# cohensbw/ElPhDynamics

Measured on AMD Instinct MI355X. Metric: cg_matvecs_per_sec, higher is better.
Workload: dtype f64; 1 GPU; BASELINE config C: Holstein square L=16 Ntau=160 (N=256, Ltau=160, Ndim=40960), un-preconditioned CG iteration, 288 right-hand sides per step on each GPU = 144 independent Markov chain(s) x 2 solve(s) each (2 = the two pseudofermion solves of one HMC force evaluation), 1 GPU(s) with their own chains; nrhs=288, chains_per_gpu=144, ndim=40960, preconditioned=False, form=workgroup-resident: K iterations of the whole batch in one launch (k_cg_wg), parallelism=gpus1xchains144

## Files before the change

elphdynamics_amd/csrc/cg_wg.hip:

```cpp

#include <algorithm>
#include <atomic>
#include <type_traits>

#include "cg_fast_common.h"

#include "cg_wg_dev.h"
#include "pgrid_dev.h"

namespace wg {

#ifdef ELPH_WG_ARRIVE
__device__ unsigned long long g_wg_arrive[4096 * 4];
__device__ unsigned long long g_wg_timeline[4096 * 4];
#define TL(k) do { if (threadIdx.x == 0 && blockIdx.x < 4096) g_wg_timeline[blockIdx.x * 4 + (k)] = (unsigned long long)wall_clock64(); } while (0)
#else
#define TL(k) do { } while (0)
#endif

struct WgRankArgs { CgBufs B; ModelDev m; WgCtl R; ShardCtl Sh; };
template <int NPL, int T, bool SSH, bool UNI, int FORM, bool SHARD, bool X0Z = false, bool RANKS = false>
__global__ void __launch_bounds__(512) k_cg_wg(CgBufs B, ModelDev m, WgCtl R, ShardCtl Sh) {
    static_assert(!RANKS || SHARD, "several ranks per launch: sharded solves only");
    unsigned bid = 0;
// ... 55 lines not shown
    double *eall = rall + (size_t)(X_REG ? 1 : 2) * W * T * HSL;
    double *el = eall + (size_t)wv * (E_SHARED ? T : T + 1) * HSL;
    double *partA = eall + (E_LDS ? (E_SHARED ? ((size_t)W * T + 1) * HSL : (size_t)W * (T + 1) * HSL) : (S_LDS ? (size_t)W * SQ_TABS * WAVE : 0)), *partB = partA + 8, *bc = partA + 16;
    double *part = partA, *tot = partA + 32, *partF = partA + 40, *rhalo = partA + 48, *zhalo = rhalo + 2 * HSL;
    double *phl = zhalo + 2 * HSL + (size_t)wv * 2 * HSL;
#define PHALO(k, q) phl[((k) ? 1 : 0) * HSL + lr + (q) * LSL]
    auto wrap = [L](int t) { return (t < 0) ? t + L : ((t >= L) ? t - L : t); };
    auto sgn = [](int t) { return (t == 0) ? -1.0 : 1.0; };
    const CgParams P = B.params;
    CgState *st2 = B.state + 2 * rhs;
    const CgState S = ld_state(st2);
    if (!SHARD && (S.done || S.seq != 0)) return;

    int sc[NPL], ss[NPL];
    bool live[NPL], own[NPL];
#pragma unroll
    for (int q = 0; q < NPL; ++q) {
        const int s = SQ ? sq_patch_site(lane, q) : (HC ? hc_site(lane, q) : (S8 ? s8_site(lane) : (GR ? grid_site(lane, q, GGX, GGY) : (HG ? hgrid_site<NPL>(lane, q, HLX, HLY) : lane + q * WAVE))));
        live[q] = (GR || HG) ? lwok : (REGX || s < N);
        own[q] = SHARD ? (live[q] && s >= Sh.own_lo && s < Sh.own_hi) : (HC ? hc_real(lane) : live[q]);
        sc[q] = live[q] ? s : N - 1;
        ss[q] = live[q] ? s : N;
    }
    double *xg = B.x + (size_t)rhs * ndim, *rg = B.r + (size_t)rhs * ndim;
    const double *Ech = m.E + (size_t)(rhs % m.nchains) * m.E_chain_stride;

    double zw[T + 1][NPL], p[T + 2][NPL], E[E_LDS ? 1 : NEJ][NPL], xr[X_REG ? T : 1][NPL];
#pragma unroll
    for (int j = 0; j < T; ++j)
#pragma unroll
        for (int q = 0; q < NPL; ++q) {
            if (lwok) rl[j * HSL + lr + q * LSL] = rg[(size_t)(t0 + j) * N + sc[q]];
            if (X_GLB) {}
            else if (X_REG) xr[X_REG ? j : 0][q] = X0Z ? 0.0 : xg[(size_t)(t0 + j) * N + sc[q]];
            else if (lwok) xl[j * HSL + lr + q * LSL] = X0Z ? 0.0 : xg[(size_t)(t0 + j) * N + sc[q]];
        }
#pragma unroll
    for (int j = 0; j < T + 2; ++j)
#pragma unroll
        for (int q = 0; q < NPL; ++q) {
            p[j][q] = rg[(size_t)wrap(t0 + j - 1) * N + sc[q]];
            if (PH_LDS && (j == 0 || j == T + 1) && lwok) PHALO(j, q) = p[j][q];
        }
#pragma unroll
    for (int j = 0; j < NEJ; ++j)
#pragma unroll
        for (int q = 0; q < NPL; ++q) {
            const double ev = Ech[(size_t)wrap(t0 + j) * m.E_tau_stride + sc[q]];
            if (E_LDS) { if (lwok) el[j * HSL + lr + q * LSL] = ev; }
            else E[E_LDS ? 0 : j][q] = ev;
        }
    unsigned ij[NE];
    Tab<NE, UNI> tab[NT];
    SqCtx<UNI> X;
    SqSsh<NSREG, S_LDS> XS;
    HcCtx XH;
    S8Ctx X8;
    GridCtx XG;
    HgCtx XHG;
    pgrid::Ctx XT;
    if constexpr (GR) {
        XG = grid_ctx(lane, GGX, GGY, m.c_uni, m.s_uni);
        if constexpr (TG) { XT = pgrid::Tri<2, 2>::make_ctx(lane, 2 * GGX, m.c_uni, m.s_uni); XG.k4 = XT.ks; }
    } else if constexpr (HG) {
        XHG = hgrid_ctx<NPL>(lane, HLX, HLY, m.c_uni, m.s_uni);
    } else if constexpr (S8) {
        X8.th = m.s_uni / m.c_uni; X8.k4 = (m.c_uni * m.c_uni) * (m.c_uni * m.c_uni);
        X8.yx = sq_patch_ycross(lane); X8.xodd = (lane >> 1) & 1;
    } else if constexpr (HC) {
        XH.th = m.s_uni / m.c_uni; XH.k3 = m.c_uni * m.c_uni * m.c_uni;
        XH.up = (lane + 16) & (WAVE - 1); XH.dn = (lane + 48) & (WAVE - 1);
    } else if constexpr (SQ && SSH) {
        ssh_chain_select(m, rhs);
        XS.yx = sq_patch_ycross(lane);
        XS.l0 = eall + (size_t)wv * SQ_TABS * WAVE + lane;
#pragma unroll
        for (int j = 0; j <= T; ++j) {
            const double *cj = m.c + (size_t)wrap(t0 + j) * m.cs_tau_stride, *sj = m.s + (size_t)wrap(t0 + j) * m.cs_tau_stride;
            SqTabS tb;
#pragma unroll
            for (int pr = 0; pr < 2; ++pr) {
                const int b0 = m.sq_bond[0 * N + sc[2 * pr]], b2 = m.sq_bond[2 * N + sc[pr]];
                tb.ci[0][pr] = cj[b0]; tb.si[0][pr] = sj[b0];
                tb.ci[1][pr] = cj[b2]; tb.si[1][pr] = sj[b2];
            }
#pragma unroll
            for (int k = 0; k < 4; ++k) {
                const int b1 = m.sq_bond[1 * N + sc[k]], b3 = m.sq_bond[3 * N + sc[k]];
                tb.cx[0][k] = cj[b1]; tb.sx[0][k] = sj[b1];
                tb.cx[1][k] = cj[b3]; tb.sx[1][k] = sj[b3];
            }
            if (S_LDS && j == 0) {
                double *d = eall + (size_t)wv * SQ_TABS * WAVE + lane;
#pragma unroll
                for (int pr = 0; pr < 2; ++pr) {
                    d[(0 + pr) * WAVE] = tb.ci[0][pr]; d[(2 + pr) * WAVE] = tb.si[0][pr];
                    d[(4 + pr) * WAVE] = tb.ci[1][pr]; d[(6 + pr) * WAVE] = tb.si[1][pr];
                }
#pragma unroll
                for (int k = 0; k < 4; ++k) {
                    d[(8 + k) * WAVE] = tb.cx[0][k]; d[(12 + k) * WAVE] = tb.sx[0][k];
                    d[(16 + k) * WAVE] = tb.cx[1][k]; d[(20 + k) * WAVE] = tb.sx[1][k];
                }
            } else {
                XS.t[S_LDS ? (j > 0 ? j - 1 : 0) : (j < NSREG ? j : 0)] = tb;
            }
        }
    } else if constexpr (SQ) {
        X.yx = sq_patch_ycross(lane);
        if constexpr (UNI) {
            X.c[0][0] = m.c_uni; X.s[0][0] = m.s_uni / m.c_uni; X.k4 = (m.c_uni * m.c_uni) * (m.c_uni * m.c_uni);
        } else {
            X.k4 = 1.0;
#pragma unroll
            for (int col = 0; col < 4; ++col)
#pragma unroll
                for (int k = 0; k < 4; ++k) {
                    const int bd = m.sq_bond[col * N + sc[k]];
                    X.c[UNI ? 0 : col][UNI ? 0 : k] = m.c[bd];
                    X.s[UNI ? 0 : col][UNI ? 0 : k] = m.s[bd];
                }
        }
    } else {
#pragma unroll
        for (int e = 0; e < NE; ++e) ij[e] = m.lp_ij[e * WAVE + lane];
        if (SSH) {
            ssh_chain_select(m, rhs);
#pragma unroll
            for (int j = 0; j < NT; ++j)
                load_tab<NE, UNI>(tab[j], m.lp_c + (size_t)wrap(t0 + j) * m.lp_tau_stride, m.lp_s + (size_t)wrap(t0 + j) * m.lp_tau_stride, lane, m);
        } else {
            load_tab<NE, UNI>(tab[0], m.lp_c, m.lp_s, lane, m);
        }
    }
#define EXPV(j, q) (E_LDS ? el[(j) * HSL + lr + (q) * LSL] : E[(SSH || E_LDS) ? 0 : (j)][q])

    constexpr size_t SLOTS_RHS = SLOTS_PER_RHS;
    u64 *const slots0 = R.slots + (size_t)rhs * 2 * SLOTS_RHS;
    u64 *const bnd0 = R.bnd + (size_t)rhs * 2 * G * 2 * HS * 2;
    const int gm = (g == 0) ? G - 1 : g - 1, gp = (g == G - 1) ? 0 : g + 1;
    double rho = S.rho, kmin = S.kmin, eps = S.eps;
    double eps0 = S.eps0, normb = S.normb;

    if (threadIdx.x == 0) { tot[5] = 1.0; if (SHARD) bc[2] = 1.0; }
    if (G > 1) {
        if (wv == 0) {
#pragma unroll
            for (int q = 0; q < NPL; ++q) if (lwok) rhalo[lr + q * LSL] = p[0][q];
        }
        if (wv == W - 1) {
#pragma unroll
            for (int q = 0; q < NPL; ++q) if (lwok) rhalo[HSL + lr + q * LSL] = p[T + 1][q];
        }
    }
    const u64 *gaddr[NPL];
    if constexpr (SHARD) {
#pragma unroll
        for (int q = 0; q < NPL; ++q) {
            const int s = ss[q];
            gaddr[q] = (s < Sh.own_lo) ? sh_ghost(Sh.mail[Sh.rank], 0, L, Sh.cap_ghost, t0, s)
                     : (s >= Sh.own_hi && s < N) ? sh_ghost(Sh.mail[Sh.rank], 1, L, Sh.cap_ghost, t0, s - Sh.own_hi) : nullptr;
        }
        double a0 = 0.0;
#pragma unroll
        for (int q = 0; q < NPL; ++q) if (own[q]) a0 += p[1][q] * p[1][q];
        a0 = wave_sum_dpp(a0);
        if (lane == 0) partA[wv] = a0;
        wg_barrier();
        if (wv == 0) {
            const double mine = wg_sum(partA, W, lane);
            sh_publish<RANKS>(Sh, 0, g, G, mine, 1u, lane);
            const u64 *none[NPL];
#pragma unroll
            for (int q = 0; q < NPL; ++q) none[q] = nullptr;
            double tot = 0.0, dummy[NPL];
            const bool ok = sh_poll<NPL, RANKS>(Sh, true, 0, G, none, 1u, lane, R, tot, dummy);
            if (lane == 0) { bc[0] = tot; if (!ok) bc[2] = 0.0; }
        }
        wg_barrier();
        if (bc[2] == 0.0) return;
        const double bb = bc[0];
        normb = sqrt(bb); eps0 = 1.0; eps = 1.0; rho = bb; kmin = 0.0;
        wg_barrier();
    }
    double rr_far = (P.tol * normb) * (P.tol * normb) * 1.000001, y_num = 4.0 * (eps0 * normb) * (eps0 * normb);
    double it_kappa = 0.17 * sqrt(P.kmax);
    constexpr bool FUSED = !SHARD && T >= 2, BSUM = SQ;
    auto uni = [](double v) __attribute__((always_inline)) {
        return __hiloint2double(__builtin_amdgcn_readfirstlane(__double2hiint(v)), __builtin_amdgcn_readfirstlane(__double2loint(v)));
    };
    if constexpr (FUSED) { rr_far = uni(rr_far); y_num = uni(y_num); it_kappa = uni(it_kappa); normb = uni(normb); eps0 = uni(eps0); }
    STAMP_DECL;
    for (long long seq = 0;; ++seq) {
        const unsigned epoch = R.epoch0 + (unsigned)seq + (SHARD ? 2u : 1u);
        const unsigned par = epoch & 1u;
        u64 *const slotsA = slots0 + (size_t)par * SLOTS_RHS, *const slotsB = slotsA + SLOTS_A;
        u64 *const bnd = bnd0 + (size_t)par * G * 2 * HS * 2;
        const size_t ghp = SHARD ? (size_t)par * 2 * L * Sh.cap_ghost * 2 : 0;
        STAMP(9);
        if (seq == 0) TL(0);
        if (seq == 1) TL(1);
        double (&w)[T + 1][NPL] = zw;
        double b_pz = 0.0, b_rz = 0.0, b_zz = 0.0, b_rr = 0.0;
        if constexpr (S8) {
#pragma unroll
            for (int k = 0; k <= T; ++k) w[k][0] = EXPV(k, 0) * p[k][0];
            s8_sweepN<T + 1, false>(w, X8);
#pragma unroll
            for (int k = 0; k <= T; ++k) w[k][0] = p[k + 1][0] - sgn(wrap(t0 + k)) * X8.k4 * w[k][0];
            double gq[T][1];
#pragma unroll
            for (int i = 0; i < T; ++i) gq[i][0] = w[i + 1][0];
            s8_sweepN<T, true>(gq, X8);
#pragma unroll
            for (int i = 0; i < T; ++i) w[i][0] = w[i][0] - sgn(wrap(t0 + i + 1)) * X8.k4 * (EXPV(i + 1, 0) * gq[i][0]);
        } else if constexpr (HC) {
#pragma unroll
            for (int k = 0; k <= T; ++k)
#pragma unroll
                for (int q = 0; q < NPL; ++q) w[k][q] = EXPV(k, q) * ((PH_LDS && k == 0) ? PHALO(0, q) : p[k][q]);
            hc_sweepN<T + 1, false>(w, XH);
#pragma unroll
            for (int k = 0; k <= T; ++k) {
                const double sg = sgn(wrap(t0 + k)) * XH.k3;
#pragma unroll
                for (int q = 0; q < NPL; ++q) w[k][q] = ((PH_LDS && k == T) ? PHALO(1, q) : p[k + 1][q]) - sg * w[k][q];
            }
            auto rev = [&](auto nb, auto j0c) __attribute__((always_inline)) {
                constexpr int NB = decltype(nb)::value, j0 = decltype(j0c)::value;
                double gq[NB][NPL];
#pragma unroll
                for (int i = 0; i < NB; ++i)
#pragma unroll
                    for (int q = 0; q < NPL; ++q) gq[i][q] = w[j0 + i + 1][q];
                hc_sweepN<NB, true>(gq, XH);
#pragma unroll
                for (int i = 0; i < NB; ++i) {
                    const double sg = sgn(wrap(t0 + j0 + i + 1)) * XH.k3;
#pragma unroll
                    for (int q = 0; q < NPL; ++q) w[j0 + i][q] = w[j0 + i][q] - sg * (EXPV(j0 + i + 1, q) * gq[i][q]);
                }
            };
            using std::integral_constant;
            if constexpr (T == 3) { rev(integral_constant<int, 2>(), integral_constant<int, 0>()); rev(integral_constant<int, 1>(), integral_constant<int, 2>()); }
            else rev(integral_constant<int, T>(), integral_constant<int, 0>());
        } else if constexpr (HG) {
#pragma unroll
            for (int k = 0; k <= T; ++k)
#pragma unroll
                for (int q = 0; q < NPL; ++q) w[k][q] = EXPV(k, q) * p[k][q];
            hgrid_sweepN<NPL, T + 1, false>(w, XHG);
#pragma unroll
            for (int k = 0; k <= T; ++k) {
                const double sg = sgn(wrap(t0 + k)) * XHG.k3;
#pragma unroll
                for (int q = 0; q < NPL; ++q) w[k][q] = p[k + 1][q] - sg * w[k][q];
            }
            double gq[T][NPL];
#pragma unroll
            for (int i = 0; i < T; ++i)
#pragma unroll
                for (int q = 0; q < NPL; ++q) gq[i][q] = w[i + 1][q];
            hgrid_sweepN<NPL, T, true>(gq, XHG);
#pragma unroll
            for (int i = 0; i < T; ++i) {
                const double sg = sgn(wrap(t0 + i + 1)) * XHG.k3;
#pragma unroll
                for (int q = 0; q < NPL; ++q) w[i][q] = w[i][q] - sg * (EXPV(i + 1, q) * gq[i][q]);
            }
        } else if constexpr (GR) {
#pragma unroll
            for (int k = 0; k <= T; ++k)
#pragma unroll
                for (int q = 0; q < 4; ++q) w[k][q] = EXPV(k, q) * p[k][q];
            if constexpr (TG) {
#pragma unroll
                for (int k = 0; k <= T; ++k) pgrid::Tri<2, 2>::apply<false>(w[k], XT);
            } else grid_sweepN<T + 1, false, (T >= 4) ? 1 : 2>(w, XG);
#pragma unroll
            for (int k = 0; k <= T; ++k) {
                const double sg = sgn(wrap(t0 + k)) * XG.k4;
#pragma unroll
                for (int q = 0; q < 4; ++q) w[k][q] = p[k + 1][q] - sg * w[k][q];
            }
            constexpr int RBG = (T >= 4) ? 2 : T;
#pragma unroll
            for (int j0 = 0; j0 < T; j0 += RBG) {
                double gq[RBG][4];
#pragma unroll
                for (int i = 0; i < RBG; ++i)
#pragma unroll
                    for (int q = 0; q < 4; ++q) gq[i][q] = w[j0 + i + 1][q];
                if constexpr (TG) {
#pragma unroll
                    for (int i = 0; i < RBG; ++i) pgrid::Tri<2, 2>::apply<true>(gq[i], XT);
                } else grid_sweepN<RBG, true, (T >= 4) ? 1 : 2>(gq, XG);
#pragma unroll
                for (int i = 0; i < RBG; ++i) {
                    const double sg = sgn(wrap(t0 + j0 + i + 1)) * XG.k4;
#pragma unroll
                    for (int q = 0; q < 4; ++q) w[j0 + i][q] = w[j0 + i][q] - sg * (EXPV(j0 + i + 1, q) * gq[i][q]);
                }
            }
        } else if constexpr (SQ) {
#pragma unroll
            for (int k = 0; k <= T; ++k)
#pragma unroll
                for (int q = 0; q < 4; ++q) w[k][q] = EXPV(k, q) * p[k][q];
            if constexpr (SSH) sq_sweepS<T + 1, false, 0>(w, XS);
            else sq_sweepN<T + 1, false, UNI>(w, X);
#pragma unroll
            for (int k = 0; k <= T; ++k) {
                const double sg = UNI ? sgn(wrap(t0 + k)) * X.k4 : sgn(wrap(t0 + k));
#pragma unroll
                for (int q = 0; q < 4; ++q) w[k][q] = p[k + 1][q] - sg * w[k][q];
            }
            constexpr int RB = (T >= 4) ? 2 : T;
#pragma unroll
            for (int j0 = 0; j0 < T; j0 += RB) {
                double gq[RB][4];
#pragma unroll
                for (int i = 0; i < RB; ++i)
#pragma unroll
                    for (int q = 0; q < 4; ++q) gq[i][q] = w[j0 + i + 1][q];
                if constexpr (SSH) sq_sweepS<RB, true, 1>(gq, XS);
                else sq_sweepN<RB, true, UNI>(gq, X);
#pragma unroll
                for (int i = 0; i < RB; ++i) {
                    const double sg = UNI ? sgn(wrap(t0 + j0 + i + 1)) * X.k4 : sgn(wrap(t0 + j0 + i + 1));
#pragma unroll
                    for (int q = 0; q < 4; ++q) w[j0 + i][q] = w[j0 + i][q] - sg * (EXPV(j0 + i + 1, q) * gq[i][q]);
                }
                if constexpr (BSUM) {
#pragma unroll
                for (int i = 0; i < RB; ++i)
#pragma unroll
                    for (int q = 0; q < 4; ++q)
                        if (own[q]) {
                            const double rv = rl[(j0 + i) * HSL + lr + q * LSL];
                            b_pz += p[j0 + i + 1][q] * w[j0 + i][q];
                            b_rz += rv * w[j0 + i][q];
                            b_zz += w[j0 + i][q] * w[j0 + i][q];
                            b_rr += rv * rv;
                        }
                }
            }
        } else {
#pragma unroll
            for (int k = 0; k <= T; ++k)
#pragma unroll
                for (int q = 0; q < NPL; ++q) slab[k * SL + lane + q * WAVE] = EXPV(k, q) * p[k][q];
            WAVE_LDS_ORDER();
            sweepN<NPL, T + 1, false, UNI, NT, SSH ? 1 : 0, 0>(slab, ij, tab, m.ncol);
#pragma unroll
            for (int k = 0; k <= T; ++k) {
                const double sg = sgn(wrap(t0 + k));
#pragma unroll
                for (int q = 0; q < NPL; ++q) w[k][q] = p[k + 1][q] - sg * slab[k * SL + lane + q * WAVE];
            }
            WAVE_LDS_ORDER();
#pragma unroll
            for (int j = 0; j < T; ++j)
#pragma unroll
                for (int q = 0; q < NPL; ++q) slab[j * SL + lane + q * WAVE] = w[j + 1][q];
            WAVE_LDS_ORDER();
            sweepN<NPL, T, true, UNI, NT, SSH ? 1 : 0, SSH ? 1 : 0>(slab, ij, tab, m.ncol);
#pragma unroll
            for (int j = 0; j < T; ++j) {
                const double sg = sgn(wrap(t0 + j + 1));
#pragma unroll
                for (int q = 0; q < NPL; ++q) w[j][q] = w[j][q] - sg * EXPV(j + 1, q) * slab[j * SL + lane + q * WAVE];
            }
            WAVE_LDS_ORDER();
        }
        double (&z)[T + 1][NPL] = zw;
        int lane_b = lane;
        if constexpr (HC && T >= 3) asm volatile("" : "+v"(lane_b));
        double rr;
        double alpha_f = 0.0;
        {
        double s_pz = b_pz, s_rz = b_rz, s_zz = b_zz, s_rr = b_rr;
        if constexpr (!BSUM) {
#pragma unroll
        for (int j = 0; j < T; ++j)
#pragma unroll
            for (int q = 0; q < NPL; ++q)
                if (own[q]) {
                    const double rv = rl[j * HSL + lr + q * LSL];
                    s_pz += p[j + 1][q] * z[j][q];
                    s_rz += rv * z[j][q];
                    s_zz += z[j][q] * z[j][q];
                    s_rr += rv * rv;
                }
        }
        {
            const double k4 = wave_sum4(s_pz, s_rz, s_zz, s_rr, lane);
            if (lane < 4) part[lane * 8 + wv] = k4;
        }
        if constexpr (X_GLB) {
#pragma unroll
            for (int j = 0; j < T; ++j)
#pragma unroll
                for (int q = 0; q < NPL; ++q) xr[X_REG ? j : 0][q] = xg[(size_t)(t0 + j) * N + sc[q]];
        }
        if constexpr (SHARD) {
            const int prev = (Sh.rank + Sh.P - 1) % Sh.P, next = (Sh.rank + 1) % Sh.P;
#pragma unroll
            for (int q = 0; q < NPL; ++q) {
                const int s = ss[q];
                const u64 bits = (u64)__double_as_longlong(z[0][q]), tag = (u64)epoch << 32;
                if (s >= Sh.own_lo && s < Sh.own_lo + Sh.n_to_prev) {
                    u64 *d = sh_ghost(Sh.mail[prev], 1, L, Sh.cap_ghost, t0, s - Sh.own_lo) + ghp;
                    st_mail<RANKS>(d, tag | (bits & 0xFFFFFFFFull)); st_mail<RANKS>(d + 1, tag | (bits >> 32));
                }
                if (s >= Sh.own_hi - Sh.n_to_next && s < Sh.own_hi) {
                    u64 *d = sh_ghost(Sh.mail[next], 0, L, Sh.cap_ghost, t0, s - (Sh.own_hi - Sh.n_to_next)) + ghp;
                    st_mail<RANKS>(d, tag | (bits & 0xFFFFFFFFull)); st_mail<RANKS>(d + 1, tag | (bits >> 32));
                }
            }
        }
        if (G > 1) {
            if (wv == 0) {
#pragma unroll
                for (int q = 0; q < NPL; ++q) {
                    st_f64_gran(bnd + (((size_t)g * 2 + 0) * HS + lane_b + q * WAVE) * 2, z[0][q], epoch);
                    if constexpr (HC && T >= 3) __builtin_amdgcn_sched_barrier(0);
                }
            }
            if (wv == W - 1) {
#pragma unroll
                for (int q = 0; q < NPL; ++q) {
                    st_f64_gran(bnd + (((size_t)g * 2 + 1) * HS + lane_b + q * WAVE) * 2, z[T - 1][q], epoch);
                    if constexpr (HC && T >= 3) __builtin_amdgcn_sched_barrier(0);
                }
            }
        }
        STAMP(0);
        wg_barrier();
        STAMP(2);
        double pap, rz, zz, rr0;
        double gz[NPL];
        if constexpr (SHARD) {
            const int rw = (W >= 3) ? 1 : 0;
            u64 *rankrec = Sh.mail[Sh.rank] + (size_t)SH_MAXREC * 2 + (size_t)par * 8 * REC4;
            bool ok = true;
            if (wv == rw) publish_rec4(slotsA, g, sum_part4(part, W, lane), epoch, lane);
            {
                const bool bw = G > 1 && (wv == 0 || wv == W - 1);
                const int th = (wv == 0) ? wrap(t0 - 1) : wrap(t0 + T);
                const u64 *bh = bw ? ((wv == 0) ? bnd + (((size_t)gm * 2 + 1) * HS) * 2 : bnd + (((size_t)gp * 2 + 0) * HS) * 2) : nullptr;
                const u64 *ga2[NPL];
#pragma unroll
                for (int q = 0; q < NPL; ++q) {
                    const int s = ss[q];
                    ga2[q] = !bw ? nullptr
                           : (s < Sh.own_lo) ? sh_ghost(Sh.mail[Sh.rank], 0, L, Sh.cap_ghost, th, s) + ghp
                           : (s >= Sh.own_hi && s < N) ? sh_ghost(Sh.mail[Sh.rank], 1, L, Sh.cap_ghost, th, s - Sh.own_hi) + ghp : nullptr;
                }
                u64 a0[NPL], a1[NPL], h0[NPL], h1[NPL], c0[NPL], c1[NPL];
                long long t_start = 0;
                for (int spin = 0;; ++spin) {
                    bool good = true;
#pragma unroll
                    for (int q = 0; q < NPL; ++q) {
                        if (gaddr[q]) { a0[q] = ld_mail<RANKS>(gaddr[q] + ghp); a1[q] = ld_mail<RANKS>(gaddr[q] + ghp + 1); }
                        if (bh) { h0[q] = ld_gran(bh + 2 * (lane + q * WAVE)); h1[q] = ld_gran(bh + 2 * (lane + q * WAVE) + 1); }
                        if (ga2[q]) { c0[q] = ld_mail<RANKS>(ga2[q]); c1[q] = ld_mail<RANKS>(ga2[q] + 1); }
                    }
#pragma unroll
                    for (int q = 0; q < NPL; ++q) {
                        if (gaddr[q]) good = good && (unsigned)(a0[q] >> 32) == epoch && (unsigned)(a1[q] >> 32) == epoch;
                        if (bh) good = good && (unsigned)(h0[q] >> 32) == epoch && (unsigned)(h1[q] >> 32) == epoch;
                        if (ga2[q]) good = good && (unsigned)(c0[q] >> 32) == epoch && (unsigned)(c1[q] >> 32) == epoch;
                    }
                    if (__all(good)) break;
                    if (poll_bail<NPL>(spin, t_start, lane, R)) { ok = false; break; }
                    __builtin_amdgcn_s_sleep(1);
                }
#pragma unroll
                for (int q = 0; q < NPL; ++q) {
                    gz[q] = gaddr[q] ? __hiloint2double((int)(unsigned)a1[q], (int)(unsigned)a0[q]) : 0.0;
                    if (bw) {
                        const double hv = ga2[q] ? __hiloint2double((int)(unsigned)c1[q], (int)(unsigned)c0[q])
                                                 : __hiloint2double((int)(unsigned)h1[q], (int)(unsigned)h0[q]);
                        zhalo[((wv == 0) ? 0 : HSL) + lr + q * LSL] = hv;
                    }
                }
            }
            if (wv == rw) {
                if (g == 0) {
                    double d0, d1, t4 = 0.0;
                    if (G <= 8) { u64 v[1] = {0}; ok = poll_rec4<1>(slotsA, G, nullptr, nullptr, epoch, lane, R, v, d0, d1) && ok; t4 = sum_rec4<1>(v, G, lane); }
                    else        { u64 v[4] = {0, 0, 0, 0}; ok = poll_rec4<4>(slotsA, G, nullptr, nullptr, epoch, lane, R, v, d0, d1) && ok; t4 = sum_rec4<4>(v, G, lane); }
                    const double mine = __shfl(t4, lane & 6, WAVE);
                    if (lane < 8 * Sh.P) {
                        const u64 bits = (u64)__double_as_longlong(mine);
                        st_mail<RANKS>(Sh.mail[lane >> 3] + (size_t)SH_MAXREC * 2 + (size_t)par * 8 * REC4 + (size_t)Sh.rank * REC4 + (lane & 7),
                               ((u64)epoch << 32) | ((lane & 1) ? (bits >> 32) : (bits & 0xFFFFFFFFull)));
                    }
                }
                u64 v[1] = {0};
                long long t_start = 0;
                for (int spin = 0;; ++spin) {
                    bool good = true;
                    if (lane < REC4 * Sh.P) { v[0] = ld_mail<RANKS>(rankrec + lane); good = (unsigned)(v[0] >> 32) == epoch; }
                    if (__all(good)) break;
                    if (poll_bail<1>(spin, t_start, lane, R)) { ok = false; break; }
                    __builtin_amdgcn_s_sleep(1);
                }
                const double t4 = sum_rec4<1>(v, Sh.P, lane);
                if (lane < 8 && !(lane & 1)) tot[lane >> 1] = t4;
            }
            if (!ok && lane == 0) tot[5] = 0.0;
            wg_barrier();
            if (tot[5] == 0.0) return;
            pap = tot[0]; rz = tot[1]; zz = tot[2]; rr0 = tot[3];
        } else if (G == 1) {
            const double t4 = sum_part4(part, W, lane);
            pap = readlane_f64(t4, 0); rz = readlane_f64(t4, 8); zz = readlane_f64(t4, 16); rr0 = readlane_f64(t4, 24);
        } else {
            constexpr int NSEG = 2 * NPL;
            const int rw = (W > NSEG) ? NSEG : ((W >= 3) ? 1 : 0);
            bool ok = true;
            double t4 = 0.0;
            if (wv == rw) publish_rec4(slotsA, g, sum_part4(part, W, lane), epoch, lane);
            for (int s0 = wv; s0 < NSEG || (s0 == wv && wv == rw); s0 += 2 * W) {
                const int s1 = s0 + W;
                const u64 *b0 = nullptr, *b1 = nullptr;
                if (s0 < NSEG) b0 = bnd + ((((s0 < NPL) ? (size_t)gm * 2 + 1 : (size_t)gp * 2 + 0) * HS) + lane_b + (size_t)(s0 % NPL) * WAVE) * 2;
                if (s1 < NSEG) b1 = bnd + ((((s1 < NPL) ? (size_t)gm * 2 + 1 : (size_t)gp * 2 + 0) * HS) + lane_b + (size_t)(s1 % NPL) * WAVE) * 2;
                const bool recs = (wv == rw && s0 == wv);
                double z0 = 0.0, z1 = 0.0;
                if (G <= 8) {
                    u64 v[1] = {0};
                    ok = poll_rec4<1>(recs ? slotsA : nullptr, G, b0, b1, epoch, lane, R, v, z0, z1) && ok;
                    if (recs) t4 = sum_rec4<1>(v, G, lane);
                } else {
                    u64 v[4] = {0, 0, 0, 0};
                    ok = poll_rec4<4>(recs ? slotsA : nullptr, G, b0, b1, epoch, lane, R, v, z0, z1) && ok;
                    if (recs) t4 = sum_rec4<4>(v, G, lane);
                }
                if (b0 && lwok) zhalo[(size_t)s0 * LSL + lr] = z0;
                if (b1 && lwok) zhalo[(size_t)s1 * LSL + lr] = z1;
                if (!ok) break;
            }
            if (wv == rw && lane < 8 && !(lane & 1)) tot[lane >> 1] = t4;
            if (!ok && lane == 0) tot[5] = 0.0;
#ifdef ELPH_WG_ARRIVE
            if (!ok && lane == 0 && blockIdx.x < 4096) g_wg_arrive[blockIdx.x * 4 + 3] = ((unsigned long long)(seq + 1) << 8) | (1ull << wv);
#endif
            wg_barrier();
            if (tot[5] == 0.0) return;
            pap = tot[0]; rz = tot[1]; zz = tot[2]; rr0 = tot[3];
        }
        STAMP(1);
        rho = rr0;
        const double alpha = FUSED ? uni(rr0 / pap) : rr0 / pap;
        if constexpr (FUSED) alpha_f = alpha;
        rr = rr0 + alpha * (alpha * zz - 2.0 * rz);
        if constexpr (!FUSED) {
#pragma unroll
        for (int j = 0; j < T; ++j)
#pragma unroll
            for (int q = 0; q < NPL; ++q) {
                const double zq = (SHARD && gaddr[q]) ? gz[q] : z[j][q];
                const double rn = rl[j * HSL + lr + q * LSL] - alpha * zq;
                if (lwok) rl[j * HSL + lr + q * LSL] = rn;
                if (X_GLB) { if (lwok) xg[(size_t)(t0 + j) * N + sc[q]] = xr[X_REG ? j : 0][q] + alpha * p[j + 1][q]; }
                else if (X_REG) xr[X_REG ? j : 0][q] += alpha * p[j + 1][q];
                else if (lwok) xl[j * HSL + lr + q * LSL] += alpha * p[j + 1][q];
            }
        if (G > 1 && (wv == 0 || wv == W - 1)) {
            double *rh = rhalo + ((wv == 0) ? 0 : HSL);
            const double *zh = zhalo + ((wv == 0) ? 0 : HSL);
#pragma unroll
            for (int q = 0; q < NPL; ++q) if (lwok) rh[lr + q * LSL] = rh[lr + q * LSL] - alpha * zh[lr + q * LSL];
        }
        STAMP(3);
        }
        if (!(rr > 1e-3 * rr0)) {
            double a = 0.0;
#pragma unroll
            for (int j = 0; j < T; ++j)
#pragma unroll
                for (int q = 0; q < NPL; ++q)
                    if (own[q]) {
                        const double rn = FUSED ? rl[j * HSL + lr + q * LSL] - alpha * z[j][q] : rl[j * HSL + lr + q * LSL];
                        a += rn * rn;
                    }
            a = wave_sum_dpp(a);
            if (lane == 0) partF[wv] = a;
            wg_barrier();
            if constexpr (SHARD) {
                if (wv == 0) {
                    sh_publish<RANKS>(Sh, 0, g, G, wg_sum(partF, W, lane), epoch, lane);
                    const u64 *none[NPL];
#pragma unroll
                    for (int q = 0; q < NPL; ++q) none[q] = nullptr;
                    double t = 0.0, dummy[NPL];
                    const bool ok = sh_poll<NPL, RANKS>(Sh, true, 0, G, none, epoch, lane, R, t, dummy);
                    if (lane == 0) { tot[4] = t; if (!ok) tot[5] = 0.0; }
                }
                wg_barrier();
                if (tot[5] == 0.0) return;
                rr = tot[4];
            } else if (G == 1) {
// ... 611 lines not shown
```

elphdynamics_amd/csrc/cg_wg_dev.h:

```cpp
#pragma once
#include "cg_fast_common.h"

namespace wg {

constexpr int MC = 4;
typedef unsigned long long u64;

template <int NPL>
__host__ __device__ constexpr int slab_len() { return NPL * WAVE + 2 * WAVE; }

struct WgCtl {
    u64 *slots;
    u64 *bnd;
    int *abort;
    unsigned epoch0;
    int G, W;
    long long timeout_ticks;
    long long fixed_iters;
    int x0_zero;
    const void *ranks = nullptr;
};

template <int NPL>
__device__ __forceinline__ void load_ij(unsigned (&ij)[MC * ((NPL + 1) / 2)], const ModelDev &m, int lane) {
#pragma unroll
    for (int e = 0; e < MC * ((NPL + 1) / 2); ++e) ij[e] = m.lp_ij[e * WAVE + lane];
}

template <int NE, bool UNI>
struct Tab {
    double c[UNI ? 1 : NE], s[UNI ? 1 : NE];
    __device__ __forceinline__ double C(int e) const { return c[UNI ? 0 : e]; }
    __device__ __forceinline__ double S(int e) const { return s[UNI ? 0 : e]; }
};

template <int NE, bool UNI>
__device__ __forceinline__ void load_tab(Tab<NE, UNI> &t, const double *lc, const double *ls, int lane, const ModelDev &m) {
    if (UNI) { t.c[0] = m.c_uni; t.s[0] = m.s_uni; return; }
#pragma unroll
    for (int e = 0; e < (UNI ? 1 : NE); ++e) { t.c[e] = lc[e * WAVE + lane]; t.s[e] = ls[e * WAVE + lane]; }
}

template <int NPL, int NS, bool REVERSE, bool UNI, int NT, int TSTRIDE, int T0>
__device__ __forceinline__ void sweepN(double *buf, const unsigned (&ij)[MC * ((NPL + 1) / 2)],
                                       const Tab<MC * ((NPL + 1) / 2), UNI> (&tabs)[NT], int ncol) {
    constexpr int PP = (NPL + 1) / 2, SL = slab_len<NPL>();
#pragma unroll
    for (int cc = 0; cc < MC; ++cc) {
        const int col = REVERSE ? MC - 1 - cc : cc;
        if (col < ncol) {
            double a0[NS][PP], a1[NS][PP];
#pragma unroll
            for (int k = 0; k < NS; ++k)
#pragma unroll
                for (int pp = 0; pp < PP; ++pp) {
                    const unsigned w = ij[col * PP + pp];
                    a0[k][pp] = buf[k * SL + (w & 0xFFFF)]; a1[k][pp] = buf[k * SL + (w >> 16)];
                }
#pragma unroll
            for (int k = 0; k < NS; ++k)
#pragma unroll
                for (int pp = 0; pp < PP; ++pp) {
                    const int e = col * PP + pp;
                    const unsigned w = ij[e];
                    const Tab<MC * ((NPL + 1) / 2), UNI> &t = tabs[TSTRIDE * k + T0];
                    buf[k * SL + (w & 0xFFFF)] = t.C(e) * a0[k][pp] + t.S(e) * a1[k][pp];
                    buf[k * SL + (w >> 16)] = t.C(e) * a1[k][pp] + t.S(e) * a0[k][pp];
                }
            WAVE_LDS_ORDER();
        }
    }
}

template <bool UNI>
struct SqCtx {
    static constexpr int ARITH = UNI ? 1 : 2;
    static constexpr bool GROUPS = true;
    double c[UNI ? 1 : 4][UNI ? 1 : 4], s[UNI ? 1 : 4][UNI ? 1 : 4];
    double k4;
    int yx;
    __device__ __forceinline__ double upd(int col, int k, double v, double t) const {
        if constexpr (UNI) return v + s[0][0] * t;
        else return __builtin_fma(s[UNI ? 0 : col][UNI ? 0 : k], t, c[UNI ? 0 : col][UNI ? 0 : k] * v);
    }
    __device__ __forceinline__ double up(int n, int col, int k, double v, double t) const { return upd(col, k, v, t); }
};

struct SqTabS {
    double ci[2][2], si[2][2];
    double cx[2][4], sx[2][4];
};
constexpr int SQ_TABS = 24;

template <int NREG, bool LDS0>
struct SqSsh {
    SqTabS t[NREG];
    const double *l0;
    int yx;
    __device__ __forceinline__ double up_set(int set, int col, int k, double v, double tv) const {
        double c, s;
        if (LDS0 && set == 0) {
            const int e = (col == 0) ? (k >> 1) : (col == 2) ? 4 + (k & 1) : (col == 1) ? 8 + k : 16 + k;
            c = l0[e * WAVE]; s = l0[(e + ((col & 1) ? 4 : 2)) * WAVE];
        } else {
            const SqTabS &T = t[LDS0 ? set - 1 : set];
            if (col == 0)      { c = T.ci[0][k >> 1]; s = T.si[0][k >> 1]; }
            else if (col == 2) { c = T.ci[1][k & 1];  s = T.si[1][k & 1]; }
            else               { c = T.cx[col >> 1][k]; s = T.sx[col >> 1][k]; }
        }
        return __builtin_fma(s, tv, c * v);
    }
};
template <int NREG, bool LDS0, int SOFF>
struct SqSshView {
    static constexpr int ARITH = 2;
    static constexpr bool GROUPS = false;
    const SqSsh<NREG, LDS0> &X;
    int yx;
    __device__ __forceinline__ double up(int n, int col, int k, double v, double t) const { return X.up_set(SOFF + n, col, k, v, t); }
};

template <int CNT, int COL, int N0, class CTX>
__device__ __forceinline__ void sq_colour(double (*v)[4], const CTX &X) {
    constexpr int DS = 0x080, VALU = 0x002, ARITH = CTX::ARITH;
    if constexpr (COL == 0) {
#pragma unroll
        for (int n = 0; n < CNT; ++n) {
            const double n0 = X.up(N0 + n, 0, 0, v[n][0], v[n][1]), n1 = X.up(N0 + n, 0, 1, v[n][1], v[n][0]);
            const double n2 = X.up(N0 + n, 0, 2, v[n][2], v[n][3]), n3 = X.up(N0 + n, 0, 3, v[n][3], v[n][2]);
            v[n][0] = n0; v[n][1] = n1; v[n][2] = n2; v[n][3] = n3;
        }
    } else if constexpr (COL == 1) {
#pragma unroll
        for (int n = 0; n < CNT; ++n) {
            const double t1 = dpp_f64<0x12E>(v[n][0]), t3 = dpp_f64<0x12E>(v[n][2]);
            const double t0 = dpp_f64<0x122>(v[n][1]), t2 = dpp_f64<0x122>(v[n][3]);
            v[n][0] = X.up(N0 + n, 1, 0, v[n][0], t0); v[n][1] = X.up(N0 + n, 1, 1, v[n][1], t1);
            v[n][2] = X.up(N0 + n, 1, 2, v[n][2], t2); v[n][3] = X.up(N0 + n, 1, 3, v[n][3], t3);
        }
    } else if constexpr (COL == 2) {
#pragma unroll
        for (int n = 0; n < CNT; ++n) {
            const double n0 = X.up(N0 + n, 2, 0, v[n][0], v[n][2]), n2 = X.up(N0 + n, 2, 2, v[n][2], v[n][0]);
            const double n1 = X.up(N0 + n, 2, 1, v[n][1], v[n][3]), n3 = X.up(N0 + n, 2, 3, v[n][3], v[n][1]);
            v[n][0] = n0; v[n][1] = n1; v[n][2] = n2; v[n][3] = n3;
        }
    } else {
        double c0[CNT], c1[CNT];
#pragma unroll
        for (int n = 0; n < CNT; ++n) { c0[n] = __shfl(v[n][0], X.yx, WAVE); c1[n] = __shfl(v[n][1], X.yx, WAVE); }
#pragma unroll
        for (int n = 0; n < CNT; ++n) {
            const double t2 = dpp_f64<0xB1>(v[n][2]), t3 = dpp_f64<0xB1>(v[n][3]);
            v[n][2] = X.up(N0 + n, 3, 2, v[n][2], t2); v[n][3] = X.up(N0 + n, 3, 3, v[n][3], t3);
        }
#pragma unroll
        for (int n = 0; n < CNT; ++n) { v[n][0] = X.up(N0 + n, 3, 0, v[n][0], c0[n]); v[n][1] = X.up(N0 + n, 3, 1, v[n][1], c1[n]); }
        if constexpr (CTX::GROUPS) {
            __builtin_amdgcn_sched_group_barrier(DS, 4 * CNT, 0);
            __builtin_amdgcn_sched_group_barrier(VALU, (4 + 4 * ARITH) * CNT, 0);
        }
    }
    __builtin_amdgcn_sched_barrier(0);
}

template <int NS, int N0, int COL, class CTX>
__device__ __forceinline__ void sq_pairs(double (&v)[NS][4], const CTX &X) {
    sq_colour<(N0 + 1 < NS) ? 2 : 1, COL, N0, CTX>(&v[N0], X);
    if constexpr (N0 + 2 < NS) sq_pairs<NS, N0 + 2, COL, CTX>(v, X);
}

template <int NS, bool REVERSE, class CTX>
__device__ __forceinline__ void sq_sweepC(double (&v)[NS][4], const CTX &X) {
    if constexpr (!REVERSE) { sq_pairs<NS, 0, 0, CTX>(v, X); sq_pairs<NS, 0, 1, CTX>(v, X); sq_pairs<NS, 0, 2, CTX>(v, X); sq_pairs<NS, 0, 3, CTX>(v, X); }
    else                    { sq_pairs<NS, 0, 3, CTX>(v, X); sq_pairs<NS, 0, 2, CTX>(v, X); sq_pairs<NS, 0, 1, CTX>(v, X); sq_pairs<NS, 0, 0, CTX>(v, X); }
}

template <int NS, bool REVERSE, bool UNI>
__device__ __forceinline__ void sq_sweepN(double (&v)[NS][4], const SqCtx<UNI> &X) { sq_sweepC<NS, REVERSE, SqCtx<UNI>>(v, X); }

template <int NS, bool REVERSE, int SOFF, int NREG, bool LDS0>
__device__ __forceinline__ void sq_sweepS(double (&v)[NS][4], const SqSsh<NREG, LDS0> &X) {
    const SqSshView<NREG, LDS0, SOFF> V{X, X.yx};
    sq_sweepC<NS, REVERSE, SqSshView<NREG, LDS0, SOFF>>(v, V);
}

constexpr int HC_NPL = 6;
__device__ __forceinline__ int hc_site(int lane, int q) {
    const int c = lane & 15, x = (c >= 2) ? ((c >= 14) ? c - 14 : c - 2) : c + 10;
    return 2 * (x + 12 * (3 * (lane >> 4) + (q >> 1))) + (q & 1);
}
__device__ __forceinline__ bool hc_real(int lane) { const int c = lane & 15; return c >= 2 && c <= 13; }
__device__ __forceinline__ int hc_src_lane(int lane) { const int c = lane & 15; return (c < 2) ? lane + 12 : ((c > 13) ? lane - 12 : lane); }

struct HcCtx {
    double th, k3;
    int up, dn;
};

template <int CNT, int COL>
__device__ __forceinline__ void hc_colour(double (*v)[HC_NPL], const HcCtx &X) {
    if constexpr (COL == 0) {
#pragma unroll
        for (int n = 0; n < CNT; ++n)
#pragma unroll
            for (int j = 0; j < 3; ++j) {
                const double a = v[n][2 * j] + X.th * v[n][2 * j + 1], b = v[n][2 * j + 1] + X.th * v[n][2 * j];
                v[n][2 * j] = a; v[n][2 * j + 1] = b;
            }
    } else if constexpr (COL == 1) {
#pragma unroll
        for (int n = 0; n < CNT; ++n) {
            double ta[3], tb[3];
#pragma unroll
            for (int j = 0; j < 3; ++j) { ta[j] = dpp_f64<0x121>(v[n][2 * j + 1]); tb[j] = dpp_f64<0x12F>(v[n][2 * j]); }
#pragma unroll
            for (int j = 0; j < 3; ++j) { v[n][2 * j] += X.th * ta[j]; v[n][2 * j + 1] += X.th * tb[j]; }
        }
    } else {
        double c0[CNT], c5[CNT];
#pragma unroll
        for (int n = 0; n < CNT; ++n) { c0[n] = __shfl(v[n][5], X.dn, WAVE); c5[n] = __shfl(v[n][0], X.up, WAVE); }
#pragma unroll
        for (int n = 0; n < CNT; ++n)
#pragma unroll
            for (int j = 0; j < 2; ++j) {
                const double b = v[n][2 * j + 1] + X.th * v[n][2 * j + 2], a = v[n][2 * j + 2] + X.th * v[n][2 * j + 1];
                v[n][2 * j + 1] = b; v[n][2 * j + 2] = a;
            }
#pragma unroll
        for (int n = 0; n < CNT; ++n) { v[n][0] += X.th * c0[n]; v[n][5] += X.th * c5[n]; }
    }
    __builtin_amdgcn_sched_barrier(0);
}

template <int NS, int N0, int COL>
__device__ __forceinline__ void hc_pairs(double (&v)[NS][HC_NPL], const HcCtx &X) {
    hc_colour<(N0 + 1 < NS) ? 2 : 1, COL>(&v[N0], X);
    if constexpr (N0 + 2 < NS) hc_pairs<NS, N0 + 2, COL>(v, X);
}

template <int NS, bool REVERSE>
__device__ __forceinline__ void hc_sweepN(double (&v)[NS][HC_NPL], const HcCtx &X) {
    if constexpr (!REVERSE) { hc_pairs<NS, 0, 0>(v, X); hc_pairs<NS, 0, 1>(v, X); hc_pairs<NS, 0, 2>(v, X); }
    else                    { hc_pairs<NS, 0, 2>(v, X); hc_pairs<NS, 0, 1>(v, X); hc_pairs<NS, 0, 0>(v, X); }
}

__device__ __forceinline__ int s8_site(int lane) { return ((lane >> 1) & 7) + 8 * (2 * (lane >> 4) + (lane & 1)); }
struct S8Ctx { double th, k4; int yx; bool xodd; };

template <int NS, bool REVERSE>
__device__ __forceinline__ void s8_sweepN(double (&v)[NS][1], const S8Ctx &X) {
#pragma unroll
    for (int cc = 0; cc < 4; ++cc) {
        const int col = REVERSE ? 3 - cc : cc;
        if (col == 0) {
#pragma unroll
            for (int n = 0; n < NS; ++n) v[n][0] += X.th * dpp_f64<0x4E>(v[n][0]);
        } else if (col == 1) {
#pragma unroll
            for (int n = 0; n < NS; ++n) {
                const double up = dpp_f64<0x12E>(v[n][0]), dn = dpp_f64<0x122>(v[n][0]);
                v[n][0] += X.th * (X.xodd ? up : dn);
            }
        } else if (col == 2) {
#pragma unroll
            for (int n = 0; n < NS; ++n) v[n][0] += X.th * dpp_f64<0xB1>(v[n][0]);
        } else {
            double t[NS];
#pragma unroll
            for (int n = 0; n < NS; ++n) t[n] = __shfl(v[n][0], X.yx, WAVE);
#pragma unroll
            for (int n = 0; n < NS; ++n) v[n][0] += X.th * t[n];
        }
        __builtin_amdgcn_sched_barrier(0);
    }
}

#ifdef ELPH_WG_STAMPS
__device__ unsigned long long g_wg_stamps[16];
#define STAMP_DECL long long _ts = wall_clock64(); unsigned long long _acc[10] = {0, 0, 0, 0, 0, 0, 0, 0, 0, 0}
#define STAMP(k) do { __builtin_amdgcn_sched_barrier(0); const long long _n = wall_clock64(); _acc[k] += (unsigned long long)(_n - _ts); _ts = _n; __builtin_amdgcn_sched_barrier(0); } while (0)
#ifndef ELPH_WG_STAMP_WAVE
#define ELPH_WG_STAMP_WAVE 0
#endif
#define STAMP_OUT(iters) do { if (rhs == 0 && g == 0 && wv == ELPH_WG_STAMP_WAVE && lane == 0) { for (int _k = 0; _k < 10; ++_k) g_wg_stamps[_k] = _acc[_k]; g_wg_stamps[10] = (unsigned long long)(iters); } } while (0)
#else
#define STAMP_DECL
#define STAMP(k)
#define STAMP_OUT(iters)
#endif

__device__ __forceinline__ void st_gran(u64 *p, u64 v) { __hip_atomic_store(p, v, __ATOMIC_RELAXED, __HIP_MEMORY_SCOPE_AGENT); }
__device__ __forceinline__ u64 ld_gran(const u64 *p) { return __hip_atomic_load(p, __ATOMIC_RELAXED, __HIP_MEMORY_SCOPE_AGENT); }
__device__ __forceinline__ void st_sc1(double *p, double v) { __hip_atomic_store(p, v, __ATOMIC_RELAXED, __HIP_MEMORY_SCOPE_AGENT); }
__device__ __forceinline__ double ld_sc1(const double *p) { return __hip_atomic_load(p, __ATOMIC_RELAXED, __HIP_MEMORY_SCOPE_AGENT); }

template <int NPL>
__device__ __forceinline__ bool poll_bail(int spin, long long &t_start, int lane, const WgCtl &R) {
    if ((spin & 31) != 31) return false;
    if (__hip_atomic_load(R.abort, __ATOMIC_RELAXED, __HIP_MEMORY_SCOPE_AGENT) != 0) return true;
    const long long now = wall_clock64();
    if (t_start == 0) { t_start = now; return false; }
    if (now - t_start > R.timeout_ticks) {
        if (lane == 0) __hip_atomic_store(R.abort, 1, __ATOMIC_RELAXED, __HIP_MEMORY_SCOPE_AGENT);
        return true;
    }
    return false;
}

__device__ __forceinline__ bool poll_records(const u64 *rec, int G, unsigned epoch, int lane, const WgCtl &R, u64 &v) {
    const bool mine = lane < 2 * G;
    u64 a = 0, b = 0, c = 0;
    if (mine) a = ld_gran(rec + lane);
    __builtin_amdgcn_s_sleep(2);
    if (mine) b = ld_gran(rec + lane);
    __builtin_amdgcn_s_sleep(2);
    if (mine) c = ld_gran(rec + lane);
    long long t_start = 0;
    for (int spin = 0;; ++spin) {
        if (__all(!mine || (unsigned)(a >> 32) == epoch)) { v = a; return true; }
        if (mine) a = ld_gran(rec + lane);
        if (__all(!mine || (unsigned)(b >> 32) == epoch)) { v = b; return true; }
        if (mine) b = ld_gran(rec + lane);
        if (__all(!mine || (unsigned)(c >> 32) == epoch)) { v = c; return true; }
        if (mine) c = ld_gran(rec + lane);
        if (poll_bail<1>(spin, t_start, lane, R)) return false;
    }
}

constexpr int REC4 = 8;
constexpr int SLOTS_A = REC4 * 32;
constexpr int SLOTS_PER_RHS = SLOTS_A + 64;

__device__ __forceinline__ void publish_rec4(u64 *slots, int g, double mine, unsigned epoch, int lane) {
    if (lane < 32 && (lane & 7) < 2) {
        const u64 bits = (u64)__double_as_longlong(mine);
        st_gran(slots + REC4 * g + 2 * (lane >> 3) + (lane & 1), ((u64)epoch << 32) | ((lane & 1) ? (bits >> 32) : (bits & 0xFFFFFFFFull)));
    }
}

template <int NL>
__device__ __forceinline__ double sum_rec4(const u64 (&v)[NL], int G, int lane) {
    double acc = 0.0;
#pragma unroll
    for (int k = 0; k < NL; ++k) {
        const int lo = (int)(unsigned)v[k];
        const int hi = __builtin_amdgcn_update_dpp(0, lo, 0xF5, 0xF, 0xF, true);
        const double val = __hiloint2double(hi, lo);
        acc += (8 * k + (lane >> 3) < G) ? val : 0.0;
    }
    acc += dpp_f64<0x128>(acc);
    acc += __shfl_xor(acc, 16, WAVE);
    acc += __shfl_xor(acc, 32, WAVE);
    return acc;
}

__device__ __forceinline__ double sum_part4(const double *part, int W, int lane) {
    double v = (lane < 32 && (lane & 7) < W) ? part[lane] : 0.0;
    v += dpp_f64<0xB1>(v);
    v += dpp_f64<0x4E>(v);
    v += dpp_f64<0x141>(v);
    return v;
}

template <int NL>
__device__ __forceinline__ bool poll_rec4(const u64 *rec, int G, const u64 *b0, const u64 *b1, unsigned epoch, int lane, const WgCtl &R,
                                          u64 (&v)[NL], double &z0, double &z1) {
    const int ngran = REC4 * G;
    u64 a0 = 0, a1 = 0, c0 = 0, c1 = 0;
    long long t_start = 0;
    for (int spin = 0;; ++spin) {
        bool ok = true;
        if (rec) {
#pragma unroll
            for (int k = 0; k < NL; ++k) if (lane + WAVE * k < ngran) v[k] = ld_gran(rec + lane + WAVE * k);
        }
        if (b0) { a0 = ld_gran(b0); a1 = ld_gran(b0 + 1); }
        if (b1) { c0 = ld_gran(b1); c1 = ld_gran(b1 + 1); }
        if (rec) {
#pragma unroll
            for (int k = 0; k < NL; ++k) if (lane + WAVE * k < ngran) ok = ok && (unsigned)(v[k] >> 32) == epoch;
        }
        if (b0) ok = ok && (unsigned)(a0 >> 32) == epoch && (unsigned)(a1 >> 32) == epoch;
        if (b1) ok = ok && (unsigned)(c0 >> 32) == epoch && (unsigned)(c1 >> 32) == epoch;
        if (__all(ok)) break;
        if (poll_bail<1>(spin, t_start, lane, R)) return false;
        __builtin_amdgcn_s_sleep(1);
    }
    z0 = __hiloint2double((int)(unsigned)a1, (int)(unsigned)a0);
    z1 = __hiloint2double((int)(unsigned)c1, (int)(unsigned)c0);
    return true;
}

__device__ __forceinline__ void st_f64_gran(u64 *g2, double v, unsigned epoch) {
    const u64 bits = (u64)__double_as_longlong(v), tag = (u64)epoch << 32;
    st_gran(g2, tag | (bits & 0xFFFFFFFFull));
    st_gran(g2 + 1, tag | (bits >> 32));
}

__device__ __forceinline__ double wave_sum_dpp(double v) {
    v += dpp_f64<0xB1>(v);
    v += dpp_f64<0x4E>(v);
    v += dpp_f64<0x141>(v);
    v += dpp_f64<0x140>(v);
    const double r0 = __hiloint2double(__builtin_amdgcn_readlane(__double2hiint(v), 0), __builtin_amdgcn_readlane(__double2loint(v), 0));
    const double r1 = __hiloint2double(__builtin_amdgcn_readlane(__double2hiint(v), 16), __builtin_amdgcn_readlane(__double2loint(v), 16));
    const double r2 = __hiloint2double(__builtin_amdgcn_readlane(__double2hiint(v), 32), __builtin_amdgcn_readlane(__double2loint(v), 32));
    const double r3 = __hiloint2double(__builtin_amdgcn_readlane(__double2hiint(v), 48), __builtin_amdgcn_readlane(__double2loint(v), 48));
    return (r0 + r1) + (r2 + r3);
}

__device__ __forceinline__ double wave_sum4(double a0, double a1, double a2, double a3, int lane) {
    const bool odd = (lane & 1) != 0, hi2 = (lane & 2) != 0;
    double k0 = odd ? a1 : a0, k1 = odd ? a3 : a2;
    const double s0 = odd ? a0 : a1, s1 = odd ? a2 : a3;
    k0 += dpp_f64<0xB1>(s0);
    k1 += dpp_f64<0xB1>(s1);
    double k = hi2 ? k1 : k0;
    const double s = hi2 ? k0 : k1;
    k += dpp_f64<0x4E>(s);
    k += dpp_f64<0x124>(k);
    k += dpp_f64<0x128>(k);
    k += __shfl_xor(k, 16, WAVE);
    k += __shfl_xor(k, 32, WAVE);
    return k;
}

__device__ __forceinline__ double readlane_f64(double v, int l) {
    const int lo = __builtin_amdgcn_readlane(__double2loint(v), l), hi = __builtin_amdgcn_readlane(__double2hiint(v), l);
    return __hiloint2double(hi, lo);
}

__device__ __forceinline__ double wg_sum(const double *part, int W, int lane) {
    const double mine = (lane < W) ? part[lane] : 0.0;
    double tot = 0.0;
#pragma unroll
    for (int i = 0; i < 8; ++i) if (i < W) tot += readlane_f64(mine, i);
    return tot;
}

__device__ __forceinline__ void wg_barrier() {
    asm volatile("s_waitcnt lgkmcnt(0)" ::: "memory");
    __builtin_amdgcn_s_barrier();
    asm volatile("" ::: "memory");
}

using ShardCtl = ElphShardCtl;
constexpr int SH_MAXREC = ELPH_SHARD_MAXREC;
constexpr size_t SH_REC_WORDS = 2 * (size_t)SH_MAXREC * 2;

__device__ __forceinline__ void st_sys(u64 *p, u64 v) { __hip_atomic_store(p, v, __ATOMIC_RELAXED, __HIP_MEMORY_SCOPE_SYSTEM); }
__device__ __forceinline__ u64 ld_sys(const u64 *p) { return __hip_atomic_load(p, __ATOMIC_RELAXED, __HIP_MEMORY_SCOPE_SYSTEM); }
template <bool LOCAL> __device__ __forceinline__ void st_mail(u64 *p, u64 v) { if constexpr (LOCAL) st_gran(p, v); else st_sys(p, v); }
template <bool LOCAL> __device__ __forceinline__ u64 ld_mail(const u64 *p) { if constexpr (LOCAL) return ld_gran(p); else return ld_sys(p); }
__device__ __forceinline__ u64 *sh_ghost(u64 *mail, int region, int L, int cap, int t, int k) {
    return mail + SH_REC_WORDS + (((size_t)region * L + t) * cap + k) * 2;
}

template <bool LOCAL = false>
__device__ __forceinline__ void sh_publish(const ShardCtl &Sh, int m, int g, int G, double mine, unsigned epoch, int lane) {
    if (lane < 2 * Sh.P) {
        const u64 bits = (u64)__double_as_longlong(mine);
        const int dest = lane >> 1, half = lane & 1;
        st_mail<LOCAL>(Sh.mail[dest] + ((size_t)m * SH_MAXREC + (size_t)Sh.rank * G + g) * 2 + half,
               ((u64)epoch << 32) | (half ? (bits >> 32) : (bits & 0xFFFFFFFFull)));
    }
}

template <int NPL, bool LOCAL = false>
__device__ __forceinline__ bool sh_poll(const ShardCtl &Sh, bool rec, int m, int G, const u64 *const (&gaddr)[NPL], unsigned epoch,
                                        int lane, const WgCtl &R, double &total, double (&gv)[NPL]) {
    constexpr int NV = 2 * SH_MAXREC / WAVE;
    const int nrec2 = 2 * Sh.P * G;
    const u64 *rbase = Sh.mail[Sh.rank] + (size_t)m * SH_MAXREC * 2;
    u64 v[NV], g0[NPL], g1[NPL];
#pragma unroll
    for (int s = 0; s < NV; ++s) v[s] = 0;
    long long t_start = 0;
    for (int spin = 0;; ++spin) {
        bool ok = true;
        if (rec) {
#pragma unroll
// ... 33 lines not shown
```

Measured before the change: 19.83 million matvec/s.

## Interleave cross-lane shuffles with sweep work in square T=4 uniform path

Adds a specialised T=4 uniform square-lattice path that splits the colour-3 cross-lane update into an issue phase (shuffles) and an apply phase, so shuffle latency overlaps with other colour sweeps, forward tails and the reverse-batch reductions. Scheduling barriers pin the interleaving order. The reverse sweep is fused with the dot-product accumulation and prefetches the next crossing. It adds many live registers and duplicates the generic path, which could lower occupancy or introduce ordering bugs if the colour sequence differs from the original.

Result: faster. 20.56 million matvec/s (median of 6 runs) (+3.6%).

```diff
diff --git a/elphdynamics_amd/csrc/cg_wg.hip b/elphdynamics_amd/csrc/cg_wg.hip
--- a/elphdynamics_amd/csrc/cg_wg.hip
+++ b/elphdynamics_amd/csrc/cg_wg.hip
@@ -381,6 +381,80 @@
                     for (int q = 0; q < 4; ++q) w[j0 + i][q] = w[j0 + i][q] - sg * (EXPV(j0 + i + 1, q) * gq[i][q]);
                 }
             }
+        } else if constexpr (SQ && !SSH && UNI && T == 4) {
+#pragma unroll
+            for (int k = 0; k <= T; ++k)
+#pragma unroll
+                for (int q = 0; q < 4; ++q) w[k][q] = EXPV(k, q) * p[k][q];
+            auto fwd_tail = [&](auto kc) __attribute__((always_inline)) {
+                constexpr int k = decltype(kc)::value;
+                const double sg = sgn(wrap(t0 + k)) * X.k4;
+#pragma unroll
+                for (int q = 0; q < 4; ++q) w[k][q] = p[k + 1][q] - sg * w[k][q];
+            };
+            using std::integral_constant;
+            using SX = SqCtx<UNI>;
+            double c0[2], c1[2], d0[2], d1[2], e0[1], e1[1];
+            sq_pairs<T + 1, 0, 0, SX>(w, X); sq_pairs<T + 1, 0, 1, SX>(w, X);
+            sq_colour<2, 2, 0, SX>(&w[0], X);
+            sq_cross_issue<2, SX>(&w[0], X, c0, c1);
+            sq_colour<2, 2, 2, SX>(&w[2], X); sq_colour<1, 2, 4, SX>(&w[4], X);
+            sq_cross_apply<2, 0, SX>(&w[0], X, c0, c1);
+            sq_cross_issue<2, SX>(&w[2], X, c0, c1);
+            fwd_tail(integral_constant<int, 0>()); fwd_tail(integral_constant<int, 1>());
+            __builtin_amdgcn_sched_barrier(0);
+            sq_cross_apply<2, 2, SX>(&w[2], X, c0, c1);
+            sq_cross_issue<1, SX>(&w[4], X, e0, e1);
+            fwd_tail(integral_constant<int, 2>());
+            __builtin_amdgcn_sched_barrier(0);
+            sq_cross_issue<2, SX>(&w[1], X, d0, d1);
+            fwd_tail(integral_constant<int, 3>());
+            __builtin_amdgcn_sched_barrier(0);
+            sq_cross_apply<1, 4, SX>(&w[4], X, e0, e1);
+            fwd_tail(integral_constant<int, 4>());
+            __builtin_amdgcn_sched_barrier(0);
+            auto rev_batch = [&](auto j0c, const double (&x0)[2], const double (&x1)[2], auto next_crossing) __attribute__((always_inline)) {
+                constexpr int j0 = decltype(j0c)::value;
+                double gq[2][4], ev[2][4], rv[2][4];
+#pragma unroll
+                for (int i = 0; i < 2; ++i)
+#pragma unroll
+                    for (int q = 0; q < 4; ++q) gq[i][q] = w[j0 + i + 1][q];
+                sq_cross_apply<2, 0, SX>(gq, X, x0, x1);
+                sq_colour<2, 2, 0, SX>(gq, X);
+#pragma unroll
+                for (int i = 0; i < 2; ++i)
+#pragma unroll
+                    for (int q = 0; q < 4; ++q) ev[i][q] = EXPV(j0 + i + 1, q);
+                __builtin_amdgcn_sched_barrier(0);
+                sq_colour<2, 1, 0, SX>(gq, X);
+                sq_colour<2, 0, 0, SX>(gq, X);
+#pragma unroll
+                for (int i = 0; i < 2; ++i) {
+                    const double sg = sgn(wrap(t0 + j0 + i + 1)) * X.k4;
+#pragma unroll
+                    for (int q = 0; q < 4; ++q) w[j0 + i][q] = w[j0 + i][q] - sg * (ev[i][q] * gq[i][q]);
+                }
+                __builtin_amdgcn_sched_barrier(0);
+#pragma unroll
+                for (int i = 0; i < 2; ++i)
+#pragma unroll
+                    for (int q = 0; q < 4; ++q) rv[i][q] = rl[(j0 + i) * HSL + lr + q * LSL];
+                __builtin_amdgcn_sched_barrier(0);
+                next_crossing();
+#pragma unroll
+                for (int i = 0; i < 2; ++i)
+#pragma unroll
+                    for (int q = 0; q < 4; ++q) {
+                        b_pz += p[j0 + i + 1][q] * w[j0 + i][q];
+                        b_rz += rv[i][q] * w[j0 + i][q];
+                        b_zz += w[j0 + i][q] * w[j0 + i][q];
+                        b_rr += rv[i][q] * rv[i][q];
+                    }
+                __builtin_amdgcn_sched_barrier(0);
+            };
+            rev_batch(integral_constant<int, 0>(), d0, d1, [&]() __attribute__((always_inline)) { sq_cross_issue<2, SX>(&w[3], X, c0, c1); });
+            rev_batch(integral_constant<int, 2>(), c0, c1, []() {});
         } else if constexpr (SQ) {
 #pragma unroll
             for (int k = 0; k <= T; ++k)
diff --git a/elphdynamics_amd/csrc/cg_wg_dev.h b/elphdynamics_amd/csrc/cg_wg_dev.h
--- a/elphdynamics_amd/csrc/cg_wg_dev.h
+++ b/elphdynamics_amd/csrc/cg_wg_dev.h
@@ -179,6 +179,23 @@
 template <int NS, bool REVERSE, bool UNI>
 __device__ __forceinline__ void sq_sweepN(double (&v)[NS][4], const SqCtx<UNI> &X) { sq_sweepC<NS, REVERSE, SqCtx<UNI>>(v, X); }
 
+template <int CNT, class CTX>
+__device__ __forceinline__ void sq_cross_issue(const double (*v)[4], const CTX &X, double (&c0)[CNT], double (&c1)[CNT]) {
+#pragma unroll
+    for (int n = 0; n < CNT; ++n) { c0[n] = __shfl(v[n][0], X.yx, WAVE); c1[n] = __shfl(v[n][1], X.yx, WAVE); }
+    __builtin_amdgcn_sched_barrier(0);
+}
+template <int CNT, int N0, class CTX>
+__device__ __forceinline__ void sq_cross_apply(double (*v)[4], const CTX &X, const double (&c0)[CNT], const double (&c1)[CNT]) {
+#pragma unroll
+    for (int n = 0; n < CNT; ++n) {
+        const double t2 = dpp_f64<0xB1>(v[n][2]), t3 = dpp_f64<0xB1>(v[n][3]);
+        v[n][2] = X.up(N0 + n, 3, 2, v[n][2], t2); v[n][3] = X.up(N0 + n, 3, 3, v[n][3], t3);
+    }
+#pragma unroll
+    for (int n = 0; n < CNT; ++n) { v[n][0] = X.up(N0 + n, 3, 0, v[n][0], c0[n]); v[n][1] = X.up(N0 + n, 3, 1, v[n][1], c1[n]); }
+    __builtin_amdgcn_sched_barrier(0);
+}
 template <int NS, bool REVERSE, int SOFF, int NREG, bool LDS0>
 __device__ __forceinline__ void sq_sweepS(double (&v)[NS][4], const SqSsh<NREG, LDS0> &X) {
     const SqSshView<NREG, LDS0, SOFF> V{X, X.yx};
```
